# akanazawa/human_dynamics

Measured on AMD Instinct MI355X. Metric: frames/sec/GPU (ResNet+temporal+SMPL, 224x224); SMPL verts max-abs-err, higher is better.
Workload: dtype f16x3

## Files before the change

human_dynamics_amd/csrc/gemm_conv.hip:

```cpp
#include <stdlib.h>
#include <string.h>
#include <type_traits>

#include "common.h"
#include "hmmr_hip.h"

struct ConvArgs {
    const void* in; const void* w; const float* scale; const float* shift;
    const void* res; void* out; void* out2; const float* scale2; const float* shift2;
    const float* pro_scale; const float* pro_shift;
    void* out_b; int ldo_b, n_split, relu_b;
    int M, K, cout, ldo, ldr;
    int Wo, HoWo, Hin, Win;
    long long in_img_stride; int in_row_stride, in_px_stride;
    int cin_log2, KH, KW, SY, SX, PY, PX;
    int res_strided; long long res_img_stride; int res_row_stride, res_px_stride;
    int relu, tiles_n, n_tiles;
    int kt_per_slice;
    long long out_slice_stride;
    int probe;
    const void* in2; int cin2, kt_split;
    int batch; long long bz_in, bz_w, bz_out, bz_res, bz_scale, bz_shift;
};

// ... 731 lines not shown
        const int r = RPP * p + r0, px = base + r;
        pptr[p] = (r < need && px >= 0 && px < a.M) ? in + (long long)px * C + lslot * EPS : nullptr;
    }
    const TA* wptr = (const TA*)a.w + (long long)(n0 + r0) * a.K + lslot * EPS;
    auto glds_patch = [&](int c, int buf) {
        char* sp = smem + OFF_P + buf * P_BYTES + wave * 1024;
#pragma unroll
        for (int p = 0; p < NPP; ++p) {
            const void* src = pptr[p] ? (const void*)(pptr[p] + c * BKE) : (const void*)g_zero_page;
            __builtin_amdgcn_global_load_lds((gptr_t)src, (lptr_t)(sp + p * (RPP * 128)), 16, 0, 0);
        }
    };
    auto glds_b = [&](int kt, int buf) {
        char* sb = smem + buf * B_BYTES + wave * 1024;
#pragma unroll
        for (int p = 0; p < PB; ++p)
            __builtin_amdgcn_global_load_lds((gptr_t)(wptr + (long long)(RPP * p) * a.K + kt * BKE),
                                             (lptr_t)(sb + p * (RPP * 128)), 16, 0, 0);
    };

    const int wm = wave / WGN, wn = wave % WGN;
    const int lr = lane & 31, lh = lane >> 5;
    const int fswb = (lr >> 1) & 7;
    const int b_row_off = (wn * TN + lr) * 128;
    int prow[FM];
    unsigned pmask[FM];
#pragma unroll
    for (int i = 0; i < FM; ++i) {
        prow[i] = wm * TM + i * 32 + lr;
        pmask[i] = patch_tap_mask(m0 + prow[i], a);
    }

    f32x16 acc[FM][FN];
#pragma unroll
    for (int i = 0; i < FM; ++i)
#pragma unroll
        for (int j = 0; j < FN; ++j)
#pragma unroll
            for (int r = 0; r < 16; ++r) acc[i][j][r] = 0.f;

    const int nc = C / BKE, nk = 9 * nc;
    frag_t fa[2][NCHK][FM], fb[2][NCHK][FN];
    auto read_piece = [&](frag_t (&da)[NCHK][FM], frag_t (&db)[NCHK][FN], int q, int t_, const char* sp_, const char* sb_) {
        const int ch = q >> 2, w_ = q & 3;
        if (w_ == 0 || w_ == 3) {
            const int i = w_ == 0 ? 0 : 1;
            const int ky = (t_ * 11) >> 5;
            const int tap_row = prow[i] + ky * W + (t_ - 3 * ky);
            const int row = ((pmask[i] >> t_) & 1u) ? tap_row : ZROW + (tap_row & 1);
            da[ch][i] = FragIO<TA>::read(sp_ + row * 128, ch, lh, (tap_row >> 1) & 7);
        } else {
            const int j = w_ - 1;
            db[ch][j] = FragIO<TA>::read(sb_ + b_row_off + j * 32 * 128, ch, lh, fswb);
        }
    };
    glds_patch(0, 0);
#pragma unroll
    for (int s_ = 0; s_ < NSB - 1; ++s_) glds_b(s_, s_);
    __builtin_amdgcn_sched_barrier(0);
    wait_vm_lgkm0<PB>();
    __builtin_amdgcn_s_barrier();
#pragma unroll
    for (int q = 0; q < 8; ++q) read_piece(fa[0], fb[0], q, 0, smem + OFF_P, smem);
    int t = 0, c = 0;
    auto step = [&](auto cur_c, int kt) {
        constexpr int CUR = decltype(cur_c)::value, NXT = CUR ^ 1;
        if (kt + 3 < nk) glds_b(kt + 3, (kt + 3) & 3);
        if (t == 0 && c + 1 < nc) glds_patch(c + 1, (c + 1) & 1);
        const int t1 = (t == 8) ? 0 : t + 1, cn = (t == 8) ? c + 1 : c;
        const char* sp1 = smem + OFF_P + (cn & 1) * P_BYTES;
        const char* sb1 = smem + ((kt + 1) & 3) * B_BYTES;
#pragma unroll
        for (int q = 0; q < 8; ++q) {
            read_piece(fa[NXT], fb[NXT], q, t1, sp1, sb1);
            const int ch = q >> 2, i = (q >> 1) & 1, j = q & 1;
            acc[i][j] = mma(fa[CUR][ch][i], fb[CUR][ch][j], acc[i][j]);
        }
        __builtin_amdgcn_sched_barrier(0);
        if (kt + 2 < nk) {
            const bool pend = t <= 1 && c + 1 < nc;
            if (kt + 3 < nk) { if (pend) wait_vm_lgkm0<PB + NPP>(); else wait_vm_lgkm0<PB>(); }
            else wait_vm_lgkm0<0>();
        } else wait_vm_lgkm0<63>();
        __builtin_amdgcn_sched_barrier(0);
        __builtin_amdgcn_s_barrier();
        __builtin_amdgcn_sched_barrier(0);
        t = t1; c = cn;
    };
    for (int kt = 0; kt < nk; kt += 2) {
        step(std::integral_constant<int, 0>{}, kt);
        if (kt + 1 < nk) step(std::integral_constant<int, 1>{}, kt + 1);
    }

    patch_epilogue<TO, BM, BN, WGM, WGN>(a, smem, acc, m0, n0, tid, wm, wn, lr, lh);
}

template <typename TA, typename TO, int NPP>
static int launch_pipe(const ConvArgs& base, hipStream_t stream) {
    ConvArgs a = base;
    const int tiles_m = (a.M + 255) / 256;
    a.tiles_n = (a.cout + 127) / 128;
    a.n_tiles = tiles_m * a.tiles_n;
    constexpr int kloop = 4 * 128 * 128 + 2 * NPP * 64 * 128, epi = 256 * 128 * 4;
    constexpr int lds = kloop > epi ? kloop : epi;
    static_assert(lds <= 160 * 1024, "LDS");
    auto kern = conv3x3_pipe_kernel<TA, TO, NPP>;
    static DeviceOnce once;
    if (const unsigned long long bit = once.due()) {
        HMMR_CHECK_HIP(hipFuncSetAttribute((const void*)kern, hipFuncAttributeMaxDynamicSharedMemorySize, 160 * 1024));
        once.mark(bit);
    }
    hipLaunchKernelGGL(kern, dim3(a.n_tiles), dim3(512), lds, stream, a);
    HMMR_CHECK_HIP(hipGetLastError());
    return 0;
}

static int patch_rows_bound(int bm, int h, int w) { (void)h; return bm + 2 * w + 2 + 2; }

template <typename TA, typename TO, int BM, int BN, int WGM, int WGN, int NPP>
static int launch_patch(const ConvArgs& base, hipStream_t stream) {
    ConvArgs a = base;
    const int tiles_m = (a.M + BM - 1) / BM;
    a.tiles_n = (a.cout + BN - 1) / BN;
    a.n_tiles = tiles_m * a.tiles_n;
    constexpr int kloop = 3 * BN * 128 + 2 * NPP * 64 * 128, epi = BM * BN * 4;
    constexpr int lds = kloop > epi ? kloop : epi;
    static_assert(lds <= 160 * 1024, "LDS");
    auto kern = conv3x3_patch_kernel<TA, TO, BM, BN, WGM, WGN, NPP>;
    static DeviceOnce once;
    if (const unsigned long long bit = once.due()) {
        HMMR_CHECK_HIP(hipFuncSetAttribute((const void*)kern, hipFuncAttributeMaxDynamicSharedMemorySize, 160 * 1024));
        once.mark(bit);
    }
    hipLaunchKernelGGL(kern, dim3(a.n_tiles), dim3(512), lds, stream, a);
    HMMR_CHECK_HIP(hipGetLastError());
    return 0;
}

template <typename TA, typename TO>
static int launch_patch_tiled(const ConvArgs& a, int tile, hipStream_t stream) {
    const int bm = tile == 10 ? 128 : 256;
    const int npp = (patch_rows_bound(bm, a.Hin, a.Win) + 63) / 64;
    if (tile == 9) {
        if (npp <= 5) return launch_patch<TA, TO, 256, 128, 4, 2, 5>(a, stream);
        if (npp <= 7) return launch_patch<TA, TO, 256, 128, 4, 2, 7>(a, stream);
    } else if (tile == 10) {
        if (npp <= 3) return launch_patch<TA, TO, 128, 256, 2, 4, 3>(a, stream);
        if (npp <= 4) return launch_patch<TA, TO, 128, 256, 2, 4, 4>(a, stream);
    } else if (tile == 11) {
        if constexpr (std::is_same<TA, bsplit_t>::value) {
            if (npp <= 5) return launch_pipe<TA, TO, 5>(a, stream);
            if (npp <= 6) return launch_pipe<TA, TO, 6>(a, stream);
        }
    } else {
        hmmr_set_error("hmmr_conv_gemm: k_order 1 runs tiles 9 / 11 (256x128) and 10 (128x256), not %d", tile);
        return -1;
    }
    hmmr_set_error("hmmr_conv_gemm: k_order 1, tile %d: a %d x %d image needs a patch of %d x 64 rows, more than LDS holds",
                   tile, a.Hin, a.Win, npp);
    return -1;
}

template <typename TA, typename TO, int BM, int BN, int WGM, int WGN, bool PRO, bool UTAP, int NSTAGE>
static int launch_cfg(const ConvArgs& base, int slices, hipStream_t stream) {
    ConvArgs a = base;
    const int tiles_m = (a.M + BM - 1) / BM;
    a.tiles_n = (a.cout + BN - 1) / BN;
    a.n_tiles = tiles_m * a.tiles_n;
    constexpr int kring = NSTAGE * (BM + BN) * 128, epi = BM * BN * 4;
    const int kloop = kring + ((PRO && NSTAGE >= 3) ? 8 * a.K : 0);
    const int lds = kloop > epi ? kloop : epi;
    if (lds > 160 * 1024) { hmmr_set_error("hmmr_conv_gemm: tile needs %d B of LDS (K = %d)", lds, a.K); return -1; }
    auto kern = conv_gemm_kernel<TA, TO, BM, BN, WGM, WGN, PRO, UTAP, NSTAGE>;
    static DeviceOnce once;
    if (const unsigned long long bit = once.due()) {
        HMMR_CHECK_HIP(hipFuncSetAttribute((const void*)kern, hipFuncAttributeMaxDynamicSharedMemorySize,
                                           NSTAGE >= 3 ? 160 * 1024 : lds));
        once.mark(bit);
    }
    constexpr int BKE_ = 8 * elem_traits<TA>::EPS;
    const int nk = a.K / BKE_;
    a.kt_per_slice = (nk + slices - 1) / slices;
    hipLaunchKernelGGL(kern, dim3(a.n_tiles, slices, a.batch), dim3(WGM * WGN * 64), lds, stream, a);
    HMMR_CHECK_HIP(hipGetLastError());
    return 0;
}

template <typename TA, typename TO, bool PRO, bool UTAP>
static int launch_tiled(const ConvArgs& a, int tile, int slices, hipStream_t stream) {
    switch (tile) {
        case 1: return launch_cfg<TA, TO, 128, 128, 2, 2, PRO, UTAP, 2>(a, slices, stream);
        case 2: return launch_cfg<TA, TO, 128, 64, 2, 2, PRO, UTAP, 2>(a, slices, stream);
        case 3: return launch_cfg<TA, TO, 64, 64, 2, 2, PRO, UTAP, 2>(a, slices, stream);
        case 5: return launch_cfg<TA, TO, 128, 128, 4, 2, PRO, UTAP, 2>(a, slices, stream);
        case 6: return launch_cfg<TA, TO, 128, 64, 4, 2, PRO, UTAP, 2>(a, slices, stream);
        case 7: return launch_cfg<TA, TO, 256, 128, 4, 2, PRO, UTAP, 3>(a, slices, stream);
        case 8: return launch_cfg<TA, TO, 128, 256, 2, 4, PRO, UTAP, 3>(a, slices, stream);
        default: hmmr_set_error("hmmr_conv_gemm: bad tile %d", tile); return -1;
    }
}

template <typename TA, typename TO>
static int launch_typed(const ConvArgs& a, int tile, int slices, hipStream_t stream) {
    if (tile == 0) {
        const long long t128 = (long long)((a.M + 127) / 128) * ((a.cout + 127) / 128);
        const long long t12864 = (long long)((a.M + 127) / 128) * ((a.cout + 63) / 64);
        if (a.cout >= 128 && a.cout % 128 == 0 && t128 * slices >= 192) tile = 5;
        else if (t12864 * slices >= 192) tile = 6;
        else tile = 3;
    }
    const bool utap = ((size_t)1 << a.cin_log2) * sizeof(TA) >= 128;
    if (a.pro_scale) {
        if (!utap) { hmmr_set_error("hmmr_conv_gemm: fused pre-activation needs cin*sizeof >= 128"); return -1; }
        return launch_tiled<TA, TO, true, true>(a, tile, slices, stream);
    }
    return utap ? launch_tiled<TA, TO, false, true>(a, tile, slices, stream)
                : launch_tiled<TA, TO, false, false>(a, tile, slices, stream);
}

template <typename TO>
__global__ __launch_bounds__(256) void splitk_reduce_kernel(const ConvArgs a0, const float* __restrict__ part,
                                                            int slices, int ldw, long long plane) {
    const ConvArgs a = batch_problem(a0, blockIdx.y);
    part += (long long)blockIdx.y * slices * plane;
    const int vpr = (a.cout + 7) / 8;
    const long long i = (long long)blockIdx.x * 256 + threadIdx.x;
    if (i >= (long long)a.M * vpr) return;
    const int m = (int)(i / vpr), n = (int)(i % vpr) * 8;
    float v[8];
    load8(part + (long long)m * ldw + n, v);
    for (int s = 1; s < slices; ++s) {
        float p[8];
        load8(part + s * plane + (long long)m * ldw + n, p);
#pragma unroll
        for (int j = 0; j < 8; ++j) v[j] += p[j];
    }
    if (a.scale && a.shift) {
        float s[8], b[8]; load8(a.scale + n, s); load8(a.shift + n, b);
#pragma unroll
        for (int j = 0; j < 8; ++j) v[j] = fmaf(v[j], s[j], b[j]);
    } else if (a.scale) {
        float s[8]; load8(a.scale + n, s);
#pragma unroll
        for (int j = 0; j < 8; ++j) v[j] *= s[j];
    } else if (a.shift) {
        float b[8]; load8(a.shift + n, b);
#pragma unroll
        for (int j = 0; j < 8; ++j) v[j] += b[j];
    }
    const bool full = (n + 8 <= a.cout);
    const TO* __restrict__ res = (const TO*)a.res;
    if (res) {
        long long ro;
        if (a.res_strided) {
            const int img = m / a.HoWo, rem = m - img * a.HoWo;
            const int oy = rem / a.Wo, ox = rem - oy * a.Wo;
            ro = (long long)img * a.res_img_stride + (long long)oy * a.res_row_stride + (long long)ox * a.res_px_stride + n;
        } else {
            ro = (long long)m * a.ldr + n;
        }
        float rr[8];
        load8(res + ro, rr);
#pragma unroll
        for (int j = 0; j < 8; ++j) v[j] += rr[j];
    }
    if (a.relu) {
#pragma unroll
        for (int j = 0; j < 8; ++j) v[j] = fmaxf(v[j], 0.f);
    }
    TO* __restrict__ out = (TO*)a.out;
    TO* __restrict__ out2 = (TO*)a.out2;
    const long long oo = (long long)m * a.ldo + n;
    if (out) {
        if (full) store8(out + oo, v);
        else store_tail(out + oo, v, a.cout - n);
    }
    if (out2) {
        float s2[8], b2[8], u[8];
        load8(a.scale2 + n, s2); load8(a.shift2 + n, b2);
#pragma unroll
        for (int j = 0; j < 8; ++j) {
            const float vr = stored_value<TO>(v[j]);
            u[j] = fmaxf(fmaf(vr, s2[j], b2[j]), 0.f);
        }
        if (full) store8(out2 + oo, u);
        else store_tail(out2 + oo, u, a.cout - n);
    }
}

extern "C" size_t hmmr_conv_splitk_workspace_bytes(int m, int cout, int split_k) {
    if (split_k <= 1 || m <= 0) return 0;
    return (size_t)split_k * (size_t)m * (size_t)((cout + 127) / 128 * 128) * sizeof(float);
}

static int ilog2_exact(int v) {
    int l = 0;
    while ((1 << l) < v) ++l;
    return ((1 << l) == v) ? l : -1;
}

int hmmr_conv3x3_stream(const hmmr_conv_desc_t* d, hipStream_t stream);
int hmmr_conv1x1_stream(const hmmr_conv_desc_t* d, hipStream_t stream);

extern "C" int hmmr_conv_gemm(const hmmr_conv_desc_t* d, void* stream) {
    HMMR_REQUIRE(d && d->in && d->w && (d->out || d->out2), "hmmr_conv_gemm: null operand");
    const int esz = d->in_dtype == HMMR_BF16 ? 2 : 4;
    const int eps = d->in_dtype == HMMR_F16X3 ? 8 : 16 / esz;
    const int cl2 = ilog2_exact(d->cin);
    HMMR_REQUIRE(cl2 >= 0 && d->cin % eps == 0, "hmmr_conv_gemm: cin=%d must be a power of two >= %d", d->cin, eps);
    const int K = d->kh * d->kw * d->cin + (d->in2 ? d->cin2 : 0);
    HMMR_REQUIRE(d->kh * d->kw <= 32, "hmmr_conv_gemm: at most 32 filter taps");
    const int bke = 128 / esz;
    HMMR_REQUIRE(K % bke == 0, "hmmr_conv_gemm: K=%d must be a multiple of %d", K, bke);
    HMMR_REQUIRE(d->out_dtype != HMMR_F16X3 || d->cout % 8 == 0,
                 "hmmr_conv_gemm: a split (f16x3) output needs cout %% 8 == 0 (rows are whole hi/lo groups)");
    HMMR_REQUIRE(d->ldo % 8 == 0, "hmmr_conv_gemm: ldo=%d must be a multiple of 8", d->ldo);
    const bool px_ok = d->in_px_stride % eps == 0 ||
                       (d->kw == 1 && d->px == 0 && (d->in_px_stride * d->sx) % eps == 0);
    HMMR_REQUIRE(px_ok && d->in_row_stride % eps == 0 && d->in_img_stride % eps == 0,
                 "hmmr_conv_gemm: input strides must keep 16-byte alignment");
    HMMR_REQUIRE(!d->res || d->res_strided || d->ldr % 8 == 0, "hmmr_conv_gemm: ldr must be a multiple of 8");
    HMMR_REQUIRE(!d->res || d->cout % 8 == 0 || (!d->res_strided && d->ldr >= (d->cout + 7) / 8 * 8),
                 "hmmr_conv_gemm: residual rows must be readable up to cout rounded up to 8");
    HMMR_REQUIRE(!d->out2 || (d->scale2 && d->shift2), "hmmr_conv_gemm: out2 needs scale2/shift2");
    HMMR_REQUIRE(!d->pro_scale == !d->pro_shift, "hmmr_conv_gemm: pro_scale and pro_shift go together");
    HMMR_REQUIRE(!d->out_b || (d->out && !d->out2 && !d->res && d->split_k <= 1 && d->n_split > 0 && d->n_split < d->cout &&
                               d->n_split % 8 == 0 && d->ldo_b % 8 == 0 && d->ldo_b >= d->cout - d->n_split),
                 "hmmr_conv_gemm: bad column split (out_b needs out, n_split %% 8 == 0, no out2 / res / split_k)");
    HMMR_REQUIRE(!d->pro_scale || !d->res, "hmmr_conv_gemm: a fused pre-activation (pro_*) cannot be combined with a residual");
    HMMR_REQUIRE(!d->pro_scale || (d->py == 0 && d->px == 0 && d->kh == 1 && d->kw == 1),
                 "hmmr_conv_gemm: the fused pre-activation is for un-padded 1x1 gathers (padding must stay zero)");
    HMMR_REQUIRE(d->tile != 8 || d->cout % 256 == 0, "hmmr_conv_gemm: tile 8 (128x256) needs cout %% 256 == 0 (filter rows are padded to 128)");
    HMMR_REQUIRE(!d->in2 || (d->kh == 1 && d->kw == 1 && d->py == 0 && d->px == 0 && d->sy == 1 && d->sx == 1 && !d->pro_scale &&
                             d->split_k <= 1 && d->cin2 > 0 && d->cin % bke == 0 && d->cin2 % bke == 0 &&
                             d->in_px_stride == d->cin && d->in_row_stride == d->win * d->cin &&
                             d->in_img_stride == (int64_t)d->hin * d->win * d->cin && d->ho == d->hin && d->wo == d->win),
                 "hmmr_conv_gemm: a second operand source (in2) needs a dense 1x1 stride-1 un-padded GEMM, cin and cin2 "
                 "multiples of the 128-byte K step, no pro_scale, no split_k");
    ConvArgs a;
    a.in = d->in; a.w = d->w; a.scale = d->scale; a.shift = d->shift; a.res = d->res;
    a.out = d->out; a.out2 = d->out2; a.scale2 = d->scale2; a.shift2 = d->shift2;
    a.pro_scale = d->pro_scale; a.pro_shift = d->pro_shift;
    a.out_b = d->out_b; a.ldo_b = d->ldo_b; a.n_split = d->n_split; a.relu_b = d->relu_b;
    a.M = d->n_img * d->ho * d->wo; a.K = K; a.cout = d->cout; a.ldo = d->ldo; a.ldr = d->ldr;
    a.Wo = d->wo; a.HoWo = d->ho * d->wo; a.Hin = d->hin; a.Win = d->win;
    a.in_img_stride = d->in_img_stride; a.in_row_stride = d->in_row_stride; a.in_px_stride = d->in_px_stride;
    a.cin_log2 = cl2; a.KH = d->kh; a.KW = d->kw; a.SY = d->sy; a.SX = d->sx; a.PY = d->py; a.PX = d->px;
    a.res_strided = d->res_strided; a.res_img_stride = d->res_img_stride;
    a.res_row_stride = d->res_row_stride; a.res_px_stride = d->res_px_stride;
    a.relu = d->relu; a.tiles_n = 0; a.n_tiles = 0;
    a.kt_per_slice = 0; a.out_slice_stride = 0; a.probe = 0;
    a.in2 = d->in2; a.cin2 = d->in2 ? d->cin2 : 0; a.kt_split = d->cin / bke;
    a.batch = d->batch > 1 ? d->batch : 1;
    a.bz_in = d->batch_in_bytes; a.bz_w = d->batch_w_bytes; a.bz_out = d->batch_out_bytes;
    a.bz_res = d->batch_res_bytes; a.bz_scale = d->batch_scale_bytes; a.bz_shift = d->batch_shift_bytes;
    HMMR_REQUIRE(a.batch == 1 || (a.batch <= 64 && !d->k_order && !d->out_b && !d->in2 && !d->pro_scale &&
                                  ((d->batch_in_bytes | d->batch_w_bytes | d->batch_out_bytes | d->batch_res_bytes | d->batch_scale_bytes | d->batch_shift_bytes) & 15) == 0),
                 "hmmr_conv_gemm: a grouped launch (batch > 1) takes up to 64 problems, strides that are multiples of 16 bytes, "
                 "and no k_order / out_b / in2 / pro_scale");
#ifdef HMMR_GEMM_PROBE
    a.probe = hmmr_debug_state()->gemm_probe;
#endif
    if (a.M <= 0) return 0;
    hipStream_t s = (hipStream_t)stream;
    if (d->k_order == 2 && d->kh == 1 && d->kw == 1) return hmmr_conv1x1_stream(d, s);
    if (d->k_order) {
        HMMR_REQUIRE((d->k_order == 1 || d->k_order == 2) && d->kh == 3 && d->kw == 3 && d->sy == 1 && d->sx == 1 && d->py == 1 && d->px == 1 &&
                     d->ho == d->hin && d->wo == d->win && d->in_px_stride == d->cin && d->in_row_stride == d->win * d->cin &&
                     d->in_img_stride == (int64_t)d->hin * d->win * d->cin && (d->cin * esz) % 128 == 0 &&
                     !d->res && !d->out2 && !d->out_b && !d->pro_scale && !d->in2 && d->split_k <= 1 && d->out && d->cout % 8 == 0,
                     "hmmr_conv_gemm: k_order 1 is for 3x3 / stride 1 / pad 1 convolutions over a dense NHWC tensor with "
                     "cin a multiple of the 128-byte K step and a scale/shift/relu epilogue (no res, out2, out_b, pro_scale, in2, split_k)");
        if (d->k_order == 2) return hmmr_conv3x3_stream(d, s);
        const bool px3 = d->in_dtype == HMMR_F16X3 && d->out_dtype == HMMR_F16X3, pbf = d->in_dtype == HMMR_BF16 && d->out_dtype == HMMR_BF16;
        HMMR_REQUIRE(px3 || pbf, "hmmr_conv_gemm: k_order 1 is built for split (f16x3) and bf16 tensors");
        const int ptile = d->tile ? d->tile : 9;
        HMMR_REQUIRE((ptile == 10 ? d->cout % 256 : d->cout % 128) == 0, "hmmr_conv_gemm: k_order 1: cout must fill the tile's columns (filter rows are padded to 128)");
        if (pbf) {
            HMMR_REQUIRE(ptile != 11, "hmmr_conv_gemm: k_order 1, tile 11 (no load segment) is written for split operands; bf16 runs tiles 9 / 10");
            return launch_patch_tiled<bf16_t, bf16_t>(a, ptile, s);
        }
        return launch_patch_tiled<bsplit_t, bsplit_t>(a, ptile, s);
    }
    const bool in16 = d->in_dtype == HMMR_BF16, in32 = d->in_dtype == HMMR_F32, inx3 = d->in_dtype == HMMR_F16X3;
    const bool out16 = d->out_dtype == HMMR_BF16, out32 = d->out_dtype == HMMR_F32, outx3 = d->out_dtype == HMMR_F16X3;
    HMMR_REQUIRE((in16 || in32 || inx3) && (out16 || out32 || outx3), "hmmr_conv_gemm: unsupported dtypes %d -> %d", d->in_dtype, d->out_dtype);
    const int nk = K / bke;
    int slices = d->split_k > 1 ? d->split_k : 1;
    if (slices > nk) slices = nk;
    slices = (nk + ((nk + slices - 1) / slices) - 1) / ((nk + slices - 1) / slices);
    if (slices > 1) {
        const int ldw = (d->cout + 127) / 128 * 128;
        const long long plane = (long long)a.M * ldw;
        HMMR_REQUIRE(d->ws && d->ws_bytes >= a.batch * hmmr_conv_splitk_workspace_bytes(a.M, d->cout, slices),
                     "hmmr_conv_gemm: split-K workspace missing or too small (a grouped launch needs batch x the planes)");
        ConvArgs p = a;
        p.bz_out = (long long)slices * plane * (long long)sizeof(float);
        p.scale = p.shift = nullptr; p.res = nullptr; p.out2 = nullptr; p.scale2 = p.shift2 = nullptr;
        p.relu = 0; p.out = d->ws; p.ldo = ldw; p.out_slice_stride = plane;
        const int rc = in16 ? launch_typed<bf16_t, float>(p, d->tile, slices, s)
                     : inx3 ? launch_typed<bsplit_t, float>(p, d->tile, slices, s)
                            : launch_typed<float, float>(p, d->tile, slices, s);
        if (rc) return rc;
        const long long nvec = (long long)a.M * ((a.cout + 7) / 8);
        const unsigned grid = (unsigned)((nvec + 255) / 256);
        const dim3 rgrid(grid, a.batch);
        if (out16) hipLaunchKernelGGL(splitk_reduce_kernel<bf16_t>, rgrid, dim3(256), 0, s, a, (const float*)d->ws, slices, ldw, plane);
        else if (outx3) hipLaunchKernelGGL(splitk_reduce_kernel<bsplit_t>, rgrid, dim3(256), 0, s, a, (const float*)d->ws, slices, ldw, plane);
        else hipLaunchKernelGGL(splitk_reduce_kernel<float>, rgrid, dim3(256), 0, s, a, (const float*)d->ws, slices, ldw, plane);
        HMMR_CHECK_HIP(hipGetLastError());
        return 0;
    }
    if (in16 && out16) return launch_typed<bf16_t, bf16_t>(a, d->tile, 1, s);
    if (in16 && out32) return launch_typed<bf16_t, float>(a, d->tile, 1, s);
    if (in32 && out32) return launch_typed<float, float>(a, d->tile, 1, s);
    if (in32 && out16) return launch_typed<float, bf16_t>(a, d->tile, 1, s);
    if (inx3 && outx3) return launch_typed<bsplit_t, bsplit_t>(a, d->tile, 1, s);
    if (inx3 && out32) return launch_typed<bsplit_t, float>(a, d->tile, 1, s);
    if (in32 && outx3) return launch_typed<float, bsplit_t>(a, d->tile, 1, s);
    hmmr_set_error("hmmr_conv_gemm: unsupported dtypes %d -> %d", d->in_dtype, d->out_dtype);
    return -1;
}
```

human_dynamics_amd/csrc/temporal.hip:

```cpp
#include "common.h"
#include "hmmr_hip.h"

#define GN_EPS 1e-6f
#define TEMPORAL_SPLIT_K_MAX 5
static inline int temporal_split_k(int dtype) { return dtype == HMMR_F16X3 ? 5 : 4; }

__device__ __forceinline__ float block_sum_256(float v, float* red) {
#pragma unroll
    for (int o = 32; o > 0; o >>= 1) v += __shfl_xor(v, o);
    __syncthreads();
    if ((threadIdx.x & 63) == 0) red[threadIdx.x >> 6] = v;
    __syncthreads();
    return red[0] + red[1] + red[2] + red[3];
}

template <typename TO>
__global__ __launch_bounds__(256) void groupnorm_relu_kernel(const float* __restrict__ x,
                                                             const float* __restrict__ gamma,
                                                             const float* __restrict__ beta,
                                                             TO* __restrict__ out, int t, int c, int groups) {
    __shared__ float red[4];
    const int cpg = c / groups;
    const int b = blockIdx.x / groups, g = blockIdx.x % groups;
    const int cnt = t * cpg;
    const float* xb = x + (long long)b * t * c + g * cpg;
    float s = 0.f;
    for (int i = threadIdx.x; i < cnt; i += 256) s += xb[(i / cpg) * c + (i % cpg)];
    const float mean = block_sum_256(s, red) / (float)cnt;
    float q = 0.f;
    for (int i = threadIdx.x; i < cnt; i += 256) {
        const float d = xb[(i / cpg) * c + (i % cpg)] - mean;
        q += d * d;
    }
    const float var = block_sum_256(q, red) / (float)cnt;
    const float rstd = rsqrtf(var + GN_EPS);
    TO* ob = out + (long long)b * t * c + g * cpg;
    const int v8 = cpg / 8;
    for (int i = threadIdx.x; i < t * v8; i += 256) {
        const int tt = i / v8, j = (i % v8) * 8;
        float xv[8], gm[8], bt[8], o[8];
        load8(xb + tt * c + j, xv); load8(gamma + g * cpg + j, gm); load8(beta + g * cpg + j, bt);
#pragma unroll
        for (int e = 0; e < 8; ++e) {
            const float gain = rstd * gm[e];
            o[e] = fmaxf((xv[e] - mean) * gain + bt[e], 0.f);
        }
        store8(ob + tt * c + j, o);
    }
}

extern "C" int hmmr_groupnorm_relu(const float* x, const float* gamma, const float* beta, int b, int t,
                                   int c, int groups, void* out, int out_dtype, void* stream) {
    HMMR_REQUIRE(x && gamma && beta && out, "hmmr_groupnorm_relu: null argument");
    HMMR_REQUIRE(b > 0 && t > 0 && groups > 0 && c % groups == 0 && (c / groups) % 8 == 0,
                 "hmmr_groupnorm_relu: bad shape (channels per group must be a multiple of 8)");
    hipStream_t s = (hipStream_t)stream;
    if (out_dtype == HMMR_BF16)
        hipLaunchKernelGGL(groupnorm_relu_kernel<bf16_t>, dim3(b * groups), dim3(256), 0, s, x, gamma, beta,
                           (bf16_t*)out, t, c, groups);
    else if (out_dtype == HMMR_F32)
        hipLaunchKernelGGL(groupnorm_relu_kernel<float>, dim3(b * groups), dim3(256), 0, s, x, gamma, beta,
                           (float*)out, t, c, groups);
    else if (out_dtype == HMMR_F16X3)
        hipLaunchKernelGGL(groupnorm_relu_kernel<bsplit_t>, dim3(b * groups), dim3(256), 0, s, x, gamma, beta,
                           (bsplit_t*)out, t, c, groups);
    else { hmmr_set_error("hmmr_groupnorm_relu: bad dtype %d", out_dtype); return -1; }
    HMMR_CHECK_HIP(hipGetLastError());
    return 0;
}

static size_t align_up(size_t v, size_t a) { return (v + a - 1) / a * a; }

extern "C" size_t hmmr_temporal_workspace_bytes(int b, int t, int dtype) {
    if (b <= 0 || t <= 0) return 0;
    const size_t m = (size_t)b * t, e = dtype == HMMR_BF16 ? 2 : 4;
    return align_up(m * 2048 * e, 256) + 3 * align_up(m * 2048 * 4, 256) +
           align_up(hmmr_conv_splitk_workspace_bytes((int)m, 2048, TEMPORAL_SPLIT_K_MAX), 256);
}

extern "C" int hmmr_temporal_fwd(const hmmr_temporal_weights_t* w, const float* phi, int b, int t,
                                 float* strips, void* ws, size_t ws_bytes, void* stream) {
    HMMR_REQUIRE(w && phi && strips && ws, "hmmr_temporal_fwd: null argument");
    HMMR_REQUIRE(b > 0 && t > 0, "hmmr_temporal_fwd: bad shape");
    HMMR_REQUIRE(w->num_blocks >= 1 && w->num_blocks <= HMMR_MAX_TEMPORAL_BLOCKS, "hmmr_temporal_fwd: bad num_blocks");
    HMMR_REQUIRE(ws_bytes >= hmmr_temporal_workspace_bytes(b, t, w->dtype), "hmmr_temporal_fwd: workspace too small");
    const int C = 2048;
    const size_t m = (size_t)b * t, e = w->dtype == HMMR_BF16 ? 2 : 4;
    char* p = (char*)ws;
    void* h = p;              p += align_up(m * C * e, 256);
    float* h1 = (float*)p;    p += align_up(m * C * 4, 256);
    float* net[2];
    net[0] = (float*)p;       p += align_up(m * C * 4, 256);
    net[1] = (float*)p;       p += align_up(m * C * 4, 256);
    void* skws = p;
    const size_t skbytes = hmmr_conv_splitk_workspace_bytes((int)m, C, TEMPORAL_SPLIT_K_MAX);
    const float* cur = phi;
    for (int i = 0; i < w->num_blocks; ++i) {
        const hmmr_temporal_block_t& B = w->block[i];
        float* dst = (i == w->num_blocks - 1) ? strips : net[i & 1];
        if (hmmr_groupnorm_relu(cur, B.gn1_gamma, B.gn1_beta, b, t, C, 32, h, w->dtype, stream)) return -2;
        hmmr_conv_desc_t d = {};
        d.in = h; d.w = B.conv1.w; d.scale = B.conv1.scale; d.shift = B.conv1.shift; d.tile = B.conv1.tile;
        d.out = h1; d.in_dtype = w->dtype; d.out_dtype = HMMR_F32;
        d.n_img = b; d.hin = t; d.win = 1; d.cin = C;
        d.in_img_stride = (int64_t)t * C; d.in_row_stride = C; d.in_px_stride = C;
        d.kh = 3; d.kw = 1; d.sy = d.sx = 1; d.py = 1; d.px = 0; d.ho = t; d.wo = 1; d.cout = C; d.ldo = C;
        d.split_k = temporal_split_k(w->dtype); d.ws = skws; d.ws_bytes = skbytes;
        if (hmmr_conv_gemm(&d, stream)) return -2;
        if (hmmr_groupnorm_relu(h1, B.gn2_gamma, B.gn2_beta, b, t, C, 32, h, w->dtype, stream)) return -2;
        d.w = B.conv2.w; d.scale = B.conv2.scale; d.shift = B.conv2.shift; d.tile = B.conv2.tile;
        d.res = cur; d.ldr = C; d.out = dst;
        if (hmmr_conv_gemm(&d, stream)) return -2;
        cur = dst;
    }
    return 0;
}

extern "C" size_t hmmr_hallucinator_workspace_bytes(int m, int dtype) {
    if (m <= 0) return 0;
    const size_t e = dtype == HMMR_BF16 ? 2 : 4;
    return 3 * align_up((size_t)m * 2048 * e, 256) +
           align_up(hmmr_conv_splitk_workspace_bytes(m, 2048, TEMPORAL_SPLIT_K_MAX), 256);
}

template <typename TO>
__global__ void hal_cast_kernel(const float* __restrict__ in, TO* __restrict__ out, long long n8) {
    const long long i = (long long)blockIdx.x * blockDim.x + threadIdx.x;
    if (i >= n8) return;
    float v[8];
    load8(in + i * 8, v);
    store8(out + i * 8, v);
}

extern "C" int hmmr_hallucinator_fwd(const hmmr_hallucinator_weights_t* w, const float* phi, int m,
                                     float* out, void* ws, size_t ws_bytes, void* stream) {
    HMMR_REQUIRE(w && phi && out && ws, "hmmr_hallucinator_fwd: null argument");
    HMMR_REQUIRE(m > 0, "hmmr_hallucinator_fwd: m must be positive");
    HMMR_REQUIRE(ws_bytes >= hmmr_hallucinator_workspace_bytes(m, w->dtype), "hmmr_hallucinator_fwd: workspace too small");
    const int C = 2048;
    const size_t e = w->dtype == HMMR_BF16 ? 2 : 4;
    char* p = (char*)ws;
    void* x = p;  p += align_up((size_t)m * C * e, 256);
    void* h1 = p; p += align_up((size_t)m * C * e, 256);
    void* h2 = p; p += align_up((size_t)m * C * e, 256);
    void* sk = p;
    const size_t skb = hmmr_conv_splitk_workspace_bytes(m, C, TEMPORAL_SPLIT_K_MAX);
    hipStream_t s = (hipStream_t)stream;
    const void* xin = phi;
    if (w->dtype != HMMR_F32) {
        const long long n8 = (long long)m * C / 8;
        if (w->dtype == HMMR_BF16)
            hipLaunchKernelGGL(hal_cast_kernel<bf16_t>, dim3((unsigned)((n8 + 255) / 256)), dim3(256), 0, s, phi, (bf16_t*)x, n8);
        else
            hipLaunchKernelGGL(hal_cast_kernel<bsplit_t>, dim3((unsigned)((n8 + 255) / 256)), dim3(256), 0, s, phi, (bsplit_t*)x, n8);
        HMMR_CHECK_HIP(hipGetLastError());
        xin = x;
    }
    auto fc = [&](const void* in, const hmmr_layer_t& l, void* o, int odt, int relu, const float* res) {
        hmmr_conv_desc_t d = {};
        d.in = in; d.w = l.w; d.scale = l.scale; d.shift = l.shift; d.out = o;
        d.in_dtype = w->dtype; d.out_dtype = odt;
        d.n_img = m; d.hin = d.win = 1; d.cin = C;
        d.in_img_stride = C; d.in_row_stride = C; d.in_px_stride = C;
        d.kh = d.kw = 1; d.sy = d.sx = 1; d.ho = d.wo = 1; d.cout = C; d.ldo = C;
        d.relu = relu; d.res = res; d.ldr = C;
        d.split_k = 4; d.ws = sk; d.ws_bytes = skb;
        return hmmr_conv_gemm(&d, s);
    };
    if (fc(xin, w->fc1, h1, w->dtype, 1, nullptr)) return -2;
    if (fc(h1, w->fc2, h2, w->dtype, 1, nullptr)) return -2;
    if (fc(h2, w->fc3, out, HMMR_F32, 0, phi)) return -2;
    return 0;
}
```

human_dynamics_amd/engine.py:

```python
from __future__ import annotations

import ctypes as C
import os
import threading
import time

import numpy as np
import torch

from . import _lib as L
from . import assets, devflags, packing

DTYPES = {"f32": L.HMMR_F32, "fp32": L.HMMR_F32, "float32": L.HMMR_F32,
          "bf16": L.HMMR_BF16, "bfloat16": L.HMMR_BF16,
          "f16x3": L.HMMR_F16X3, "split": L.HMMR_F16X3}
DTYPE_NAMES = {L.HMMR_F32: "f32", L.HMMR_BF16: "bf16", L.HMMR_F16X3: "f16x3"}
DEFAULT_DTYPE = "f16x3"
TILE_TABLES = os.path.join(os.path.dirname(os.path.abspath(__file__)), "tile_tables.json")


def set_debug(stem_route=0, stem_no_conv1=0, gemm_probe=0, smpl_blend_mfma=0, ief_no_group=0, pair_min_pixels=0, pair_two_tile_min=0, pair_form=0):
    d = L.Debug()
    d.stem_route, d.stem_no_conv1, d.gemm_probe = int(stem_route), int(stem_no_conv1), int(gemm_probe)
    d.smpl_blend_mfma, d.ief_no_group, d.pair_min_pixels = int(smpl_blend_mfma), int(ief_no_group), int(pair_min_pixels)
    d.pair_two_tile_min, d.pair_form = int(pair_two_tile_min), int(pair_form)
    L.load().hmmr_set_debug(C.byref(d))


def _debug_from_env():
    e = devflags.get("STEM")
    c1 = devflags.get("STEM_C1")
    probe = int(devflags.get("GEMM_PROBE") or 0)
    if e or c1 == "0" or probe or _debug_from_env.was_set:
        set_debug(stem_route={"u": 1, "f": 2}.get(e[:1], 0), stem_no_conv1=int(c1 == "0"), gemm_probe=probe)
        _debug_from_env.was_set = bool(e or c1 == "0" or probe)


_debug_from_env.was_set = False


def _dt(d):
    if isinstance(d, str):
        if d == "bf16x3":
            import warnings
            warnings.warn("dtype 'bf16x3' is now 'f16x3' (split operands with fp16 halves since round 3)", DeprecationWarning, stacklevel=3)
            d = "f16x3"
        if d not in DTYPES:
            raise ValueError("unknown operand mode %r: use one of %s" % (d, ", ".join(sorted(set(DTYPES)))))
        return DTYPES[d]
    return int(d)


class _Workspace(object):

    def __init__(self, device):
        self.device, self.buf = device, None

    def get(self, nbytes):
        if self.buf is None or self.buf.numel() < nbytes:
            self.buf = torch.empty(int(nbytes), dtype=torch.uint8, device=self.device)
        return self.buf


class HmmrEngine(object):

    def __init__(self, weights, smpl, dtype=DEFAULT_DTYPE, device="cuda:0", num_conv_layers=3,
                 delta_t_values=(-5, 5), joint_type="cocoplus", resnet_chunk=0,
                 temporal_dtype=None, ief_dtype=None, autotune=True, fold_sc=None, fuse_tail=None, patch_3x3=None,
                 unit_pair=None, b1_stream=None, b1_unit=None, stem_conv1=True, stream_1x1=None):
        self.lib = L.load()
        _debug_from_env()
        if not torch.cuda.is_available():
            raise L.HmmrError("HmmrEngine needs a HIP device (torch.cuda.is_available() is False)")
        self.device = torch.device(device)
        torch.cuda.set_device(self.device)
        self.dtype = _dt(dtype)
        self.temporal_dtype = self.dtype if temporal_dtype is None else _dt(temporal_dtype)
        self.ief_dtype = self.dtype if ief_dtype is None else _dt(ief_dtype)
        self.resnet_chunk = int(devflags.get("RESNET_CHUNK") or resnet_chunk)
        self.store = packing.DeviceStore(self.device)
        self.num_conv_layers = num_conv_layers
        self.delta_keys = sorted(int(d) for d in delta_t_values)
        fuse = tuple(b for b in devflags.get("FUSE_PREACT").split(",") if b)
        tail = {"0": False, "1": True}.get(devflags.get("FUSE_TAIL"), devflags.get("FUSE_TAIL"))
        if fuse_tail is not None:
            tail = fuse_tail
        fsc = {"0": False, "1": True}.get(devflags.get("FUSE_SC"), "all")
        pfirst = devflags.get("PREACT_FIRST") != "0"
        fold = {"0": False, "1": True}.get(devflags.get("FOLD_SC"), None) if fold_sc is None else fold_sc
        w = weights if weights is not None else {}
        for name, v in w.items():
            a_ = np.asarray(v)
            if a_.dtype.kind == "f" and not np.isfinite(a_).all():
                raise ValueError("variable %r holds %d non-finite value(s)" % (name, int((~np.isfinite(a_)).sum())))
        self.rw = (packing.pack_resnet(w, self.dtype, self.store, fuse_preact_blocks=fuse, fuse_tail=tail, fuse_sc=fsc,
                                       fuse_preact_first=pfirst, fold_sc=fold,
                                       patch_3x3=int(devflags.get("PATCH_3X3")) if patch_3x3 is None else patch_3x3,
                                       unit_pair=({"0": False, "1": True}.get(devflags.get("UNIT_PAIR"), devflags.get("UNIT_PAIR"))
                                                  if unit_pair is None else unit_pair),
                                       b1_stream=(devflags.get("B1_STREAM") == "1") if b1_stream is None else b1_stream,
                                       b1_unit=(devflags.get("B1_UNIT") == "1") if b1_unit is None else b1_unit,
                                       stem_conv1=stem_conv1,
                                       stream_1x1=(devflags.get("STREAM_1X1") == "1") if stream_1x1 is None else stream_1x1)
                   if "resnet_v2_50/conv1/weights" in w else None)
        self.tw = (packing.pack_temporal(w, self.temporal_dtype, self.store, num_conv_layers)
                   if assets.temporal_scopes(0)[1] + "/weights" in w else None)
        self.hw = packing.pack_hallucinator(w, self.temporal_dtype, self.store)
        if "single_view_ief/3D_module/fc1/weights" in w and "mean_param" in w:
            self.iw, self.reg_keys = packing.pack_ief(w, self.ief_dtype, self.store, self.delta_keys)
        else:
            self.iw, self.reg_keys = None, [0]
        all_f32 = (self.dtype, self.temporal_dtype, self.ief_dtype) == (L.HMMR_F32,) * 3
        self.sc = packing.pack_smpl(smpl, self.store, joint_type, split=not all_f32) if smpl is not None else None
        self.num_kps = self.sc.num_kps if self.sc is not None else assets.NUM_KPS
        self.num_verts = self.sc.num_verts if self.sc is not None else assets.NUM_VERTS
        self._ws = {k: _Workspace(self.device) for k in ("resnet", "temporal", "ief", "smpl", "hal")}
        at = devflags.get("AUTOTUNE")
        self.autotune = False if (not autotune or at == "0") else ("force" if (autotune == "force" or at == "force") else True)
        self._tiles, self._shipped = {}, set()
        self.tune_log = []
        self._tile_cache = devflags.get("TILE_CACHE")
        sources = []
        if self.autotune != "force" and devflags.get("TILE_TABLE") != "0" and os.path.exists(TILE_TABLES):
            sources.append((TILE_TABLES, True))
        if self._tile_cache and os.path.exists(self._tile_cache):
            sources.append((self._tile_cache, False))
        for path, shipped in sources:
            import json
            for key, tab in json.load(open(path)).items():
                if key.startswith("_"):
                    continue
                dt, nt = key.split(":")
                if int(dt) == self.dtype:
                    self._tiles[int(nt)] = {(int(k.split(":")[0]), k.split(":")[1]): int(v) for k, v in tab.items()}
                    if shipped:
                        self._shipped.add(int(nt))
        self.resnet_streams = int(devflags.get("RESNET_STREAMS"))
        self._side_streams = []

    @staticmethod
    def _need(packed, names):
        if packed is None:
            raise L.HmmrError("the loaded weights have no %s variables: this stage was not packed" % names)

    def _stream(self):
        return torch.cuda.current_stream(self.device).cuda_stream

    _carried_flags = {}

    def run_flags(self, clear=False):
        key = (self.device.type, self.device.index)
        v = self._device_flags(clear) | HmmrEngine._carried_flags.get(key, 0)
        if clear:
            HmmrEngine._carried_flags.pop(key, None)
        return v

    def _device_flags(self, clear):
        torch.cuda.synchronize(self.device)
        with torch.cuda.device(self.device):
            v = C.c_uint(0)
            L.check(self.lib.hmmr_run_flags(C.byref(v), int(bool(clear))), "hmmr_run_flags")
        return int(v.value)

    def flag_scope(self):
        return _FlagScope(self)

    def to_device(self, a, dtype=torch.float32):
        if isinstance(a, torch.Tensor):
            return a.to(self.device, dtype).contiguous()
        return torch.from_numpy(np.ascontiguousarray(a)).to(self.device).to(dtype).contiguous()

    _TUNE_TILES = tuple(int(t) for t in devflags.get("TUNE_TILES").split(","))
    _TUNE_MIN_FRAMES = 32
    _SPLIT_MIN_FRAMES = 176

    def _resnet_layers(self):
        out, slot = [], 3
        for u in range(L.RESNET_UNITS):
            names = (["shortcut"] if self.rw.unit[u].shortcut.w else []) + ["conv1", "conv2", "conv3"]
            for nm in names:
                out.append((slot, u, nm))
                slot += 1
        return out

    def _layer_of(self, u, nm):
        U = self.rw.unit[u]
        if nm == "conv3" and U.c3sc.w:
            return U.c3sc
        return getattr(U, nm)

    @staticmethod
    def _tile_for(lay, cand, cout, dtype=None, nm="conv2"):
        if lay.k_order == 2 and nm != "conv2":
            t = {5: 22, 6: 23, 3: 24, 1: 25, 2: 26, 4: 29}.get(cand, cand if (22 <= cand <= 26 or cand == 29) else 0)
            return 0 if (nm == "conv3" and t in (22, 23, 29)) else t
        if lay.k_order == 2:
            if cout == 64:
                return {5: 19, 6: 20}.get(cand, cand if cand in (19, 20) else 0)
            t = {5: 13, 6: 14, 3: 15, 1: 16, 2: 17, 7: 18, 8: 12, 11: 21, 4: 27, 9: 28}.get(cand, cand if (12 <= cand <= 18 or cand in (21, 27, 28)) else 0)
            return 0 if (t in (21, 27, 28) and dtype == L.HMMR_BF16) else t
        if lay.k_order:
            cand = {7: 9, 8: 10}.get(cand, cand)
            if cand == 11 and dtype == L.HMMR_BF16:
                return 0
            return cand if (cand in (9, 11) and cout % 128 == 0) or (cand == 10 and cout % 256 == 0) else 0
        if cand not in (1, 2, 3, 5, 6, 7, 8) or (cand in (1, 5, 7) and cout % 128) or (cand == 8 and cout % 256):
            return 0
        return cand

    def _layer_cout(self, u, nm):
        U = self.rw.unit[u]
        if nm == "shortcut" and U.sc_c1.w:
            return U.depth + U.base
        return U.base if nm in ("conv1", "conv2") else U.depth

    def _set_tiles(self, table):
        for (u, nm), t in table.items():
            self._layer_of(u, nm).tile = self._tile_for(self._layer_of(u, nm), int(t), self._layer_cout(u, nm), self.dtype, nm)

    def _needs_tuning(self, nt):
        if not self.autotune or nt < self._TUNE_MIN_FRAMES or nt in self._tiles or torch.cuda.is_current_stream_capturing():
            return False
        if len(self.tune_log) >= 8:
            return False
        if self.autotune == "force":
            return True
        return not any(max(k, nt) <= 1.3 * min(k, nt) for k in self._tiles)

    def _tune_resnet(self, images, n, n_zero, ws_key="resnet", reps=3):
        layers = self._resnet_layers()
        t_start = time.perf_counter()
        nt = n + n_zero
        nbytes = self.lib.hmmr_resnet50_workspace_bytes(nt, self.dtype)
        ws = self._ws.setdefault(ws_key, _Workspace(self.device)).get(nbytes)
        phi = torch.empty((nt, 2048), dtype=torch.float32, device=self.device)
        src = images.data_ptr() if n else None
        best = {}
        for cand in (0,) + self._TUNE_TILES:
            for slot, u, nm in layers:
                lay = self._layer_of(u, nm)
                lay.tile = self._tile_for(lay, cand, self._layer_cout(u, nm), self.dtype, nm)
            t = None
            for rep in range(reps):
                pm = (C.c_float * L.RESNET_PROF_SLOTS)()
                L.check(self.lib.hmmr_resnet50_fwd(C.byref(self.rw), src, n, n_zero, phi.data_ptr(), ws.data_ptr(),
                                                   nbytes, self._stream(), pm), "hmmr_resnet50_fwd")
                cur = np.frombuffer(pm, dtype=np.float32).copy()
                t = cur if (t is None or rep == 0) else np.minimum(t, cur)
            for slot, u, nm in layers:
                tile = self._layer_of(u, nm).tile
                if (u, nm) not in best or t[slot] < best[(u, nm)][0] * 0.98:
                    best[(u, nm)] = (float(t[slot]), tile)
        table = {k: v[1] for k, v in best.items()}
        self.tune_log.append((nt, round((time.perf_counter() - t_start) * 1e3, 1)))
        if self._tile_cache:
            import json
            old = json.load(open(self._tile_cache)) if os.path.exists(self._tile_cache) else {}
            old["%d:%d" % (self.dtype, nt)] = {"%d:%s" % k: v for k, v in table.items()}
            json.dump(old, open(self._tile_cache, "w"))
        return table

    def _resnet_pass(self, images, n, n_zero, phi, ws_key, prof=False, tune=True):
        nt = n + n_zero
        table = None
        if tune and nt >= self._TUNE_MIN_FRAMES:
            if self._needs_tuning(nt):
                self._tiles[nt] = self._tune_resnet(images, n, n_zero, ws_key)
            if self._tiles:
                table = self._tiles[min(self._tiles, key=lambda k: abs(k - nt))]
        if table is not None:
            self._set_tiles(table)
        elif self._tiles:
            self._set_tiles({k: 0 for k in next(iter(self._tiles.values()))})
        nbytes = self.lib.hmmr_resnet50_workspace_bytes(nt, self.dtype)
        ws = self._ws.setdefault(ws_key, _Workspace(self.device)).get(nbytes)
        pm = (C.c_float * L.RESNET_PROF_SLOTS)() if prof else None
        L.check(self.lib.hmmr_resnet50_fwd(C.byref(self.rw), images.data_ptr() if n else None, n, n_zero,
                                           phi.data_ptr(), ws.data_ptr(), nbytes, self._stream(), pm),
                "hmmr_resnet50_fwd")
        return np.frombuffer(pm, dtype=np.float32).astype(np.float64) if prof else None

    def resnet_cuts(self, n, parts=None):
        parts = self.resnet_streams if parts is None else int(parts)
        if parts < 2 or n < self._SPLIT_MIN_FRAMES or self.resnet_chunk > 0:
            return [0, n]
        return [(i * n) // parts for i in range(parts + 1)]

    def resnet(self, images, prof=False, n_zero=0, out=None, ws_key="resnet", parts=None):
        self._need(self.rw, "resnet_v2_50/*")
        images = self.to_device(images)
        n = images.shape[0]
        assert n == 0 or tuple(images.shape[1:]) == (224, 224, 3), images.shape
        nt = n + n_zero
        if out is not None:
            assert out.is_cuda and out.dtype == torch.float32 and out.shape == (nt, 2048) and out.is_contiguous()
        phi = out if out is not None else torch.empty((nt, 2048), dtype=torch.float32, device=self.device)
        if self.resnet_chunk > 0:
            chunk, i = self.resnet_chunk, 0
            prof_tot = np.zeros(L.RESNET_PROF_SLOTS, np.float64) if prof else None
            while i < nt:
                c_real = max(0, min(chunk, n - i))
                c_zero = min(chunk - c_real, nt - i - c_real) if i + c_real >= n else 0
                pm = self._resnet_pass(images[i:i + c_real], c_real, c_zero, phi[i:i + c_real + c_zero], "resnet",
                                       prof, tune=False)
                if prof:
                    prof_tot += pm
                i += c_real + c_zero
            return (phi, prof_tot) if prof else phi
        parts = self.resnet_streams if parts is None else int(parts)
        if prof or parts < 2 or n < self._SPLIT_MIN_FRAMES or torch.cuda.is_current_stream_capturing():
            pm = self._resnet_pass(images, n, n_zero, phi, ws_key, prof)
            return (phi, pm) if prof else phi
        cur = torch.cuda.current_stream(self.device)
        self.side_stream(parts - 1)
        cuts = [(i * n) // parts for i in range(parts + 1)]
        if self.autotune:
            for i in range(parts):
                ni, nz = cuts[i + 1] - cuts[i], (n_zero if i == parts - 1 else 0)
                if self._needs_tuning(ni + nz):
                    self._tiles[ni + nz] = self._tune_resnet(images[cuts[i]:cuts[i + 1]], ni, nz, "resnet%d" % i)
        for i in range(parts):
            side = self._side_streams[i]
            side.wait_stream(cur)
            with torch.cuda.stream(side):
                nz = n_zero if i == parts - 1 else 0
                self._resnet_pass(images[cuts[i]:cuts[i + 1]], cuts[i + 1] - cuts[i], nz,
                                  phi[cuts[i]:cuts[i + 1] + nz], "resnet%d" % i)
        for i in range(parts):
# ... 355 lines not shown
```

Measured before the change: 39650.

## Fuse split-K reduction and epilogue into temporal groupnorm kernel

In the temporal encoder, the split-K conv GEMMs that feed a groupnorm no longer launch their own reduce kernel. The groupnorm kernel sums the partial planes itself, applies scale, shift and residual, writes the trunk output when needed, and stages the group tile in LDS for the statistics passes. This removes one kernel launch and one fp32 round trip through global memory per conv. In exchange it adds dynamic LDS use per block, which can lower occupancy, and the fused path is limited to a maximum LDS size and can be turned off with a debug flag.

```diff
diff --git a/human_dynamics_amd/csrc/gemm_conv.hip b/human_dynamics_amd/csrc/gemm_conv.hip
--- a/human_dynamics_amd/csrc/gemm_conv.hip
+++ b/human_dynamics_amd/csrc/gemm_conv.hip
@@ -1057,7 +1057,21 @@
 int hmmr_conv3x3_stream(const hmmr_conv_desc_t* d, hipStream_t stream);
 int hmmr_conv1x1_stream(const hmmr_conv_desc_t* d, hipStream_t stream);
 
-extern "C" int hmmr_conv_gemm(const hmmr_conv_desc_t* d, void* stream) {
+struct SplitkPlanes { const float* part; int slices, ldw; long long plane; };
+static int conv_gemm_impl(const hmmr_conv_desc_t* d, void* stream, SplitkPlanes* planes);
+
+extern "C" int hmmr_conv_gemm(const hmmr_conv_desc_t* d, void* stream) { return conv_gemm_impl(d, stream, nullptr); }
+
+int hmmr_conv_gemm_planes(const hmmr_conv_desc_t* d, hipStream_t stream, const float** part, int* slices, int* ldw, long long* plane) {
+    HMMR_REQUIRE(d && d->batch <= 1 && !d->relu && !d->out2 && !d->res_strided && d->out_dtype == HMMR_F32,
+                 "hmmr_conv_gemm_planes: an fp32 output without batch / relu / out2 / strided residual");
+    SplitkPlanes p = {nullptr, 0, 0, 0};
+    const int rc = conv_gemm_impl(d, (void*)stream, &p);
+    *part = p.part; *slices = p.slices; *ldw = p.ldw; *plane = p.plane;
+    return rc;
+}
+
+static int conv_gemm_impl(const hmmr_conv_desc_t* d, void* stream, SplitkPlanes* planes) {
     HMMR_REQUIRE(d && d->in && d->w && (d->out || d->out2), "hmmr_conv_gemm: null operand");
     const int esz = d->in_dtype == HMMR_BF16 ? 2 : 4;
     const int eps = d->in_dtype == HMMR_F16X3 ? 8 : 16 / esz;
@@ -1157,6 +1171,7 @@
                      : inx3 ? launch_typed<bsplit_t, float>(p, d->tile, slices, s)
                             : launch_typed<float, float>(p, d->tile, slices, s);
         if (rc) return rc;
+        if (planes) { planes->part = (const float*)d->ws; planes->slices = slices; planes->ldw = ldw; planes->plane = plane; return 0; }
         const long long nvec = (long long)a.M * ((a.cout + 7) / 8);
         const unsigned grid = (unsigned)((nvec + 255) / 256);
         const dim3 rgrid(grid, a.batch);
diff --git a/human_dynamics_amd/csrc/temporal.hip b/human_dynamics_amd/csrc/temporal.hip
--- a/human_dynamics_amd/csrc/temporal.hip
+++ b/human_dynamics_amd/csrc/temporal.hip
@@ -1,5 +1,7 @@
 #include "common.h"
 #include "hmmr_hip.h"
+
+int hmmr_conv_gemm_planes(const hmmr_conv_desc_t* d, hipStream_t stream, const float** part, int* slices, int* ldw, long long* plane);
 
 #define GN_EPS 1e-6f
 #define TEMPORAL_SPLIT_K_MAX 5
@@ -14,32 +16,80 @@
     return red[0] + red[1] + red[2] + red[3];
 }
 
-template <typename TO>
+struct GnPlanes {
+    const float* part; long long plane; int slices, ldw;
+    const float* scale; const float* shift;
+    const float* res; int ldr;
+    float* trunk;
+};
+
+template <typename TO, bool PLANES>
 __global__ __launch_bounds__(256) void groupnorm_relu_kernel(const float* __restrict__ x,
                                                              const float* __restrict__ gamma,
                                                              const float* __restrict__ beta,
-                                                             TO* __restrict__ out, int t, int c, int groups) {
+                                                             TO* __restrict__ out, int t, int c, int groups, const GnPlanes pl) {
     __shared__ float red[4];
+    extern __shared__ __attribute__((aligned(16))) float xs[];
     const int cpg = c / groups;
     const int b = blockIdx.x / groups, g = blockIdx.x % groups;
     const int cnt = t * cpg;
-    const float* xb = x + (long long)b * t * c + g * cpg;
+    const int v8 = cpg / 8;
+    const float* xb;
+    int ldx;
+    if constexpr (PLANES) {
+        for (int i = threadIdx.x; i < t * v8; i += 256) {
+            const int tt = i / v8, j = (i % v8) * 8, n = g * cpg + j;
+            const long long m = (long long)b * t + tt;
+            float v[8];
+            load8(pl.part + m * pl.ldw + n, v);
+            for (int s = 1; s < pl.slices; ++s) {
+                float p[8];
+                load8(pl.part + s * pl.plane + m * pl.ldw + n, p);
+#pragma unroll
+                for (int e = 0; e < 8; ++e) v[e] += p[e];
+            }
+            if (pl.scale && pl.shift) {
+                float sc[8], sh[8]; load8(pl.scale + n, sc); load8(pl.shift + n, sh);
+#pragma unroll
+                for (int e = 0; e < 8; ++e) v[e] = fmaf(v[e], sc[e], sh[e]);
+            } else if (pl.scale) {
+                float sc[8]; load8(pl.scale + n, sc);
+#pragma unroll
+                for (int e = 0; e < 8; ++e) v[e] *= sc[e];
+            } else if (pl.shift) {
+                float sh[8]; load8(pl.shift + n, sh);
+#pragma unroll
+                for (int e = 0; e < 8; ++e) v[e] += sh[e];
+            }
+            if (pl.res) {
+                float rr[8];
+                load8(pl.res + m * pl.ldr + n, rr);
+#pragma unroll
+                for (int e = 0; e < 8; ++e) v[e] += rr[e];
+            }
+            if (pl.trunk) store8(pl.trunk + m * c + n, v);
+            store8(xs + tt * cpg + j, v);
+        }
+        __syncthreads();
+        xb = xs; ldx = cpg;
+    } else {
+        xb = x + (long long)b * t * c + g * cpg; ldx = c;
+    }
     float s = 0.f;
-    for (int i = threadIdx.x; i < cnt; i += 256) s += xb[(i / cpg) * c + (i % cpg)];
+    for (int i = threadIdx.x; i < cnt; i += 256) s += xb[(i / cpg) * ldx + (i % cpg)];
     const float mean = block_sum_256(s, red) / (float)cnt;
     float q = 0.f;
     for (int i = threadIdx.x; i < cnt; i += 256) {
-        const float d = xb[(i / cpg) * c + (i % cpg)] - mean;
+        const float d = xb[(i / cpg) * ldx + (i % cpg)] - mean;
         q += d * d;
     }
     const float var = block_sum_256(q, red) / (float)cnt;
     const float rstd = rsqrtf(var + GN_EPS);
     TO* ob = out + (long long)b * t * c + g * cpg;
-    const int v8 = cpg / 8;
     for (int i = threadIdx.x; i < t * v8; i += 256) {
         const int tt = i / v8, j = (i % v8) * 8;
         float xv[8], gm[8], bt[8], o[8];
-        load8(xb + tt * c + j, xv); load8(gamma + g * cpg + j, gm); load8(beta + g * cpg + j, bt);
+        load8(xb + tt * ldx + j, xv); load8(gamma + g * cpg + j, gm); load8(beta + g * cpg + j, bt);
 #pragma unroll
         for (int e = 0; e < 8; ++e) {
             const float gain = rstd * gm[e];
@@ -49,24 +99,33 @@
     }
 }
 
+#define GN_PLANES_MAX_LDS (48 * 1024)
+
+static int groupnorm_relu_launch(const float* x, const GnPlanes* pl, const float* gamma, const float* beta, int b, int t,
+                                 int c, int groups, void* out, int out_dtype, hipStream_t s) {
+    HMMR_REQUIRE(b > 0 && t > 0 && groups > 0 && c % groups == 0 && (c / groups) % 8 == 0,
+                 "hmmr_groupnorm_relu: bad shape (channels per group must be a multiple of 8)");
+    const dim3 grid(b * groups), block(256);
+    const size_t lds = (size_t)t * (c / groups) * sizeof(float);
+    const GnPlanes none = {};
+    if (out_dtype == HMMR_BF16) {
+        if (pl) hipLaunchKernelGGL((groupnorm_relu_kernel<bf16_t, true>), grid, block, lds, s, x, gamma, beta, (bf16_t*)out, t, c, groups, *pl);
+        else hipLaunchKernelGGL((groupnorm_relu_kernel<bf16_t, false>), grid, block, 0, s, x, gamma, beta, (bf16_t*)out, t, c, groups, none);
+    } else if (out_dtype == HMMR_F32) {
+        if (pl) hipLaunchKernelGGL((groupnorm_relu_kernel<float, true>), grid, block, lds, s, x, gamma, beta, (float*)out, t, c, groups, *pl);
+        else hipLaunchKernelGGL((groupnorm_relu_kernel<float, false>), grid, block, 0, s, x, gamma, beta, (float*)out, t, c, groups, none);
+    } else if (out_dtype == HMMR_F16X3) {
+        if (pl) hipLaunchKernelGGL((groupnorm_relu_kernel<bsplit_t, true>), grid, block, lds, s, x, gamma, beta, (bsplit_t*)out, t, c, groups, *pl);
+        else hipLaunchKernelGGL((groupnorm_relu_kernel<bsplit_t, false>), grid, block, 0, s, x, gamma, beta, (bsplit_t*)out, t, c, groups, none);
+    } else { hmmr_set_error("hmmr_groupnorm_relu: bad dtype %d", out_dtype); return -1; }
+    HMMR_CHECK_HIP(hipGetLastError());
+    return 0;
+}
+
 extern "C" int hmmr_groupnorm_relu(const float* x, const float* gamma, const float* beta, int b, int t,
                                    int c, int groups, void* out, int out_dtype, void* stream) {
     HMMR_REQUIRE(x && gamma && beta && out, "hmmr_groupnorm_relu: null argument");
-    HMMR_REQUIRE(b > 0 && t > 0 && groups > 0 && c % groups == 0 && (c / groups) % 8 == 0,
-                 "hmmr_groupnorm_relu: bad shape (channels per group must be a multiple of 8)");
-    hipStream_t s = (hipStream_t)stream;
-    if (out_dtype == HMMR_BF16)
-        hipLaunchKernelGGL(groupnorm_relu_kernel<bf16_t>, dim3(b * groups), dim3(256), 0, s, x, gamma, beta,
-                           (bf16_t*)out, t, c, groups);
-    else if (out_dtype == HMMR_F32)
-        hipLaunchKernelGGL(groupnorm_relu_kernel<float>, dim3(b * groups), dim3(256), 0, s, x, gamma, beta,
-                           (float*)out, t, c, groups);
-    else if (out_dtype == HMMR_F16X3)
-        hipLaunchKernelGGL(groupnorm_relu_kernel<bsplit_t>, dim3(b * groups), dim3(256), 0, s, x, gamma, beta,
-                           (bsplit_t*)out, t, c, groups);
-    else { hmmr_set_error("hmmr_groupnorm_relu: bad dtype %d", out_dtype); return -1; }
-    HMMR_CHECK_HIP(hipGetLastError());
-    return 0;
+    return groupnorm_relu_launch(x, nullptr, gamma, beta, b, t, c, groups, out, out_dtype, (hipStream_t)stream);
 }
 
 static size_t align_up(size_t v, size_t a) { return (v + a - 1) / a * a; }
@@ -84,7 +143,7 @@
     HMMR_REQUIRE(b > 0 && t > 0, "hmmr_temporal_fwd: bad shape");
     HMMR_REQUIRE(w->num_blocks >= 1 && w->num_blocks <= HMMR_MAX_TEMPORAL_BLOCKS, "hmmr_temporal_fwd: bad num_blocks");
     HMMR_REQUIRE(ws_bytes >= hmmr_temporal_workspace_bytes(b, t, w->dtype), "hmmr_temporal_fwd: workspace too small");
-    const int C = 2048;
+    const int C = 2048, G = 32;
     const size_t m = (size_t)b * t, e = w->dtype == HMMR_BF16 ? 2 : 4;
     char* p = (char*)ws;
     void* h = p;              p += align_up(m * C * e, 256);
@@ -94,11 +153,24 @@
     net[1] = (float*)p;       p += align_up(m * C * 4, 256);
     void* skws = p;
     const size_t skbytes = hmmr_conv_splitk_workspace_bytes((int)m, C, TEMPORAL_SPLIT_K_MAX);
+    hipStream_t s = (hipStream_t)stream;
+    const bool gn_reduces = !hmmr_debug_state()->reserved[2] && (size_t)t * (C / G) * sizeof(float) <= GN_PLANES_MAX_LDS;
+    GnPlanes pend = {};
+    auto conv = [&](const hmmr_conv_desc_t& d, bool consumer_follows) -> int {
+        pend = GnPlanes{};
+        if (!(gn_reduces && consumer_follows)) return hmmr_conv_gemm(&d, stream);
+        const float* part; int slices, ldw; long long plane;
+        if (hmmr_conv_gemm_planes(&d, s, &part, &slices, &ldw, &plane)) return -2;
+        if (slices) pend = GnPlanes{part, plane, slices, ldw, d.scale, d.shift, (const float*)d.res, d.ldr, nullptr};
+        return 0;
+    };
     const float* cur = phi;
     for (int i = 0; i < w->num_blocks; ++i) {
         const hmmr_temporal_block_t& B = w->block[i];
-        float* dst = (i == w->num_blocks - 1) ? strips : net[i & 1];
-        if (hmmr_groupnorm_relu(cur, B.gn1_gamma, B.gn1_beta, b, t, C, 32, h, w->dtype, stream)) return -2;
+        const bool last = i == w->num_blocks - 1;
+        float* dst = last ? strips : net[i & 1];
+        if (pend.part) pend.trunk = (float*)cur;
+        if (groupnorm_relu_launch(cur, pend.part ? &pend : nullptr, B.gn1_gamma, B.gn1_beta, b, t, C, G, h, w->dtype, s)) return -2;
         hmmr_conv_desc_t d = {};
         d.in = h; d.w = B.conv1.w; d.scale = B.conv1.scale; d.shift = B.conv1.shift; d.tile = B.conv1.tile;
         d.out = h1; d.in_dtype = w->dtype; d.out_dtype = HMMR_F32;
@@ -106,11 +178,11 @@
         d.in_img_stride = (int64_t)t * C; d.in_row_stride = C; d.in_px_stride = C;
         d.kh = 3; d.kw = 1; d.sy = d.sx = 1; d.py = 1; d.px = 0; d.ho = t; d.wo = 1; d.cout = C; d.ldo = C;
         d.split_k = temporal_split_k(w->dtype); d.ws = skws; d.ws_bytes = skbytes;
-        if (hmmr_conv_gemm(&d, stream)) return -2;
-        if (hmmr_groupnorm_relu(h1, B.gn2_gamma, B.gn2_beta, b, t, C, 32, h, w->dtype, stream)) return -2;
+        if (conv(d, true)) return -2;
+        if (groupnorm_relu_launch(h1, pend.part ? &pend : nullptr, B.gn2_gamma, B.gn2_beta, b, t, C, G, h, w->dtype, s)) return -2;
         d.w = B.conv2.w; d.scale = B.conv2.scale; d.shift = B.conv2.shift; d.tile = B.conv2.tile;
         d.res = cur; d.ldr = C; d.out = dst;
-        if (hmmr_conv_gemm(&d, stream)) return -2;
+        if (conv(d, !last)) return -2;
         cur = dst;
     }
     return 0;
diff --git a/human_dynamics_amd/engine.py b/human_dynamics_amd/engine.py
--- a/human_dynamics_amd/engine.py
+++ b/human_dynamics_amd/engine.py
@@ -19,11 +19,13 @@
 TILE_TABLES = os.path.join(os.path.dirname(os.path.abspath(__file__)), "tile_tables.json")
 
 
-def set_debug(stem_route=0, stem_no_conv1=0, gemm_probe=0, smpl_blend_mfma=0, ief_no_group=0, pair_min_pixels=0, pair_two_tile_min=0, pair_form=0):
+def set_debug(stem_route=0, stem_no_conv1=0, gemm_probe=0, smpl_blend_mfma=0, ief_no_group=0, pair_min_pixels=0, pair_two_tile_min=0, pair_form=0,
+              temporal_reduce_launch=0):
     d = L.Debug()
     d.stem_route, d.stem_no_conv1, d.gemm_probe = int(stem_route), int(stem_no_conv1), int(gemm_probe)
     d.smpl_blend_mfma, d.ief_no_group, d.pair_min_pixels = int(smpl_blend_mfma), int(ief_no_group), int(pair_min_pixels)
     d.pair_two_tile_min, d.pair_form = int(pair_two_tile_min), int(pair_form)
+    d.reserved[2] = int(temporal_reduce_launch)
     L.load().hmmr_set_debug(C.byref(d))
 
 
```

Result: no change. 39740, median of 6 (+0.2%).
